# MartijnAB/guacamole

Hardware: AMD Instinct MI355X
Metric: pileup loci/sec at 30x WGS; achieved HBM GB/s vs roofline (higher is better)
Workload: dtype u8; 1 GPU; germline-threshold, synthetic 30x chr20-length shard per GPU (configs[1]); genome_loci=63025519, visited_loci_per_gpu=63025483, reads_per_gpu=12612887, contigs_per_gpu=1, read_len=150, threshold=8, parallelism=loci-sharded x1

## Files before the change

### guacamole_amd/csrc/gq_bamdev.hip

```cpp
#include <hip/hip_runtime.h>
#include <hipcub/hipcub.hpp>

#include <fcntl.h>
#include <sys/mman.h>
#include <sys/stat.h>
#include <unistd.h>

#include <zlib.h>

#include <chrono>
#include <climits>
#include <cstring>
#include <atomic>
#include <map>
#include <memory>
#include <mutex>
#include <string>
#include <thread>
#include <vector>

#include "gq_host.h"

using namespace gq;

// ... 1756 lines not shown
  (void)rehops;
  b->scanned = true;
  *sizes = b->sizes;
  return GQ_OK;
}

gq_status gq_bam_dev_reads(gq_bam_dev *b, const uint8_t *class_sample, int32_t n_samples, const uint32_t *sample_hash,
                           gq_dev_reads **out, float *fill_ms) {
  if (!b || !class_sample || !out) return set_err(GQ_E_ARG, "gq_bam_dev_reads: null argument");
  if (!b->scanned) return set_err(GQ_E_ARG, "gq_bam_dev_reads before gq_bam_dev_scan");
  if (n_samples < 1 || n_samples > 8) return set_err(GQ_E_ARG, "n_samples must be in [1, 8]");
  gq_ctx *c = b->ctx;
  HIP_TRY(hipSetDevice(c->device));
  auto t0 = std::chrono::steady_clock::now();
  const int64_t n = b->n_keep;
  const int32_t n_ref = (int32_t)b->names.size();
  if (n_ref <= 0) return set_err(GQ_E_ARG, "bad read-set sizes");
  std::unique_ptr<gq_dev_reads> dr(new gq_dev_reads());
  gq_dev_reads *d = dr.get();
  d->ctx = c;
  auto alloc = [&](size_t bytes, void **p) -> hipError_t {
    *p = nullptr;
    hipError_t e = hipMalloc(p, std::max(bytes, (size_t)16));
    if (e == hipSuccess) d->owned.push_back(*p);
    return e;
  };
  struct Guard {
    gq_dev_reads *d;
    ~Guard() {
      if (d)
        for (void *p : d->owned) (void)hipFree(p);
    }
  } guard{d};
  FillOut F{};
  void *p;
  DevBuf contig, ekey, cls, tmp, flag;
  const size_t n0 = (size_t)std::max<int64_t>(n, 1);
  HIP_TRY(contig.ensure(sizeof(int32_t) * n0));
  HIP_TRY(ekey.ensure(sizeof(uint64_t) * n0));
  F.contig = (int32_t *)contig.p;
  F.end_key = (uint64_t *)ekey.p;
  HIP_TRY(alloc(sizeof(int32_t) * n0, &p)); F.start = (int32_t *)p;
  HIP_TRY(alloc(sizeof(int32_t) * n0, &p)); F.end = (int32_t *)p;
  HIP_TRY(alloc(n0, &p)); F.mapq = (uint8_t *)p;
  HIP_TRY(alloc(n0, &p)); F.flags = (uint8_t *)p;
  HIP_TRY(alloc(n0, &p)); F.sample = (uint8_t *)p;
  HIP_TRY(alloc(sizeof(int64_t) * n0, &p)); F.seq_off = (int64_t *)p;
  HIP_TRY(alloc(sizeof(int32_t) * n0, &p)); F.seq_len = (int32_t *)p;
  HIP_TRY(alloc(sizeof(int64_t) * n0, &p)); F.cigar_off = (int64_t *)p;
  HIP_TRY(alloc(sizeof(int32_t) * n0, &p)); F.n_cigar = (int32_t *)p;
  HIP_TRY(alloc(sizeof(int64_t) * n0, &p)); F.md_off = (int64_t *)p;
  HIP_TRY(alloc(sizeof(int32_t) * n0, &p)); F.n_md = (int32_t *)p;
  HIP_TRY(alloc(sizeof(uint16_t) * n0, &p)); F.n_mismatch = (uint16_t *)p;
  HIP_TRY(alloc((size_t)b->seq_bytes + kSeqPad, &p)); F.seq = (uint8_t *)p;
  HIP_TRY(hipMemsetAsync(F.seq + b->seq_bytes, 0, kSeqPad, c->stream));
  HIP_TRY(alloc((size_t)b->seq_bytes + kSeqPad, &p)); F.qual = (uint8_t *)p;
  HIP_TRY(hipMemsetAsync(F.qual + b->seq_bytes, 0, kSeqPad, c->stream));
  HIP_TRY(alloc(sizeof(uint32_t) * (size_t)std::max<int64_t>(b->cigar_len, 1), &p)); F.cigar = (uint32_t *)p;
  HIP_TRY(alloc(sizeof(uint32_t) * (size_t)std::max<int64_t>(b->md_events, 1), &p)); F.md_ev = (uint32_t *)p;
  int32_t *pmax;
  HIP_TRY(alloc(sizeof(int32_t) * n0, &p)); pmax = (int32_t *)p;
  int64_t *begin;
  HIP_TRY(alloc(sizeof(int64_t) * (size_t)(n_ref + 1), &p)); begin = (int64_t *)p;
  const int n_cls = 256;
  HIP_TRY(cls.ensure(n_cls));
  HIP_TRY(hipMemsetAsync(cls.p, 0, n_cls, c->stream));
  HIP_TRY(hipMemcpyAsync(cls.p, class_sample, 255, hipMemcpyHostToDevice, c->stream));
  if (b->n_rec) {
    hipLaunchKernelGGL(rec_fill, dim3(grid(b->n_rec * 16, 256)), dim3(256), 0, c->stream, (const uint8_t *)b->out.p,
                       (const int64_t *)b->rec.p, b->n_rec, (const RecInfo *)b->info.p, (const int64_t *)b->kidx.p,
                       (const int64_t *)b->seq_o.p, (const int64_t *)b->cig_o.p, (const int64_t *)b->md_o.p,
                       (const uint8_t *)cls.p, F);
    HIP_TRY(hipGetLastError());
  }
  HIP_TRY(flag.ensure(sizeof(int)));
  HIP_TRY(hipMemsetAsync(flag.p, 0, sizeof(int), c->stream));
  hipLaunchKernelGGL(reads_order, dim3(grid(n + 1, 256)), dim3(256), 0, c->stream, (const int32_t *)F.contig,
                     (const int32_t *)F.start, n, n_ref, begin, (int *)flag.p);
  HIP_TRY(hipGetLastError());
  if (n) {
    size_t tb = 0;
    HIP_TRY(hipcub::DeviceScan::InclusiveScan(nullptr, tb, F.end_key, F.end_key, U64Max(), (int)n, c->stream));
    HIP_TRY(tmp.ensure(tb));
    HIP_TRY(hipcub::DeviceScan::InclusiveScan(tmp.p, tb, F.end_key, F.end_key, U64Max(), (int)n, c->stream));
    hipLaunchKernelGGL(low32, dim3(grid(n, 256)), dim3(256), 0, c->stream, (const uint64_t *)F.end_key, n, pmax);
    HIP_TRY(hipGetLastError());
  }
  int unsorted = 0;
  d->contig_read_begin.assign((size_t)n_ref + 1, 0);
  HIP_TRY(hipMemcpyAsync(&unsorted, flag.p, sizeof(int), hipMemcpyDeviceToHost, c->stream));
  HIP_TRY(hipMemcpyAsync(d->contig_read_begin.data(), begin, sizeof(int64_t) * (size_t)(n_ref + 1),
                         hipMemcpyDeviceToHost, c->stream));
  HIP_TRY(hipStreamSynchronize(c->stream));
  if (unsorted)
    return set_err(GQ_E_UNSORTED, "the BAM's kept reads are not sorted by (contig, start) (the host loader sorts them)");
  DevReads &R = d->d;
  R.n_reads = n;
  R.n_contigs = n_ref;
  R.n_samples = n_samples;
  R.contig_read_begin = begin;
  R.start = F.start;
  R.end = F.end;
  R.pmax_end = pmax;
  R.mapq = F.mapq;
  R.flags = F.flags;
  R.sample = F.sample;
  R.seq_off = F.seq_off;
  R.seq_len = F.seq_len;
  R.cigar_off = F.cigar_off;
  R.n_cigar = F.n_cigar;
  R.md_off = F.md_off;
  R.n_md = F.n_md;
  R.n_mismatch = F.n_mismatch;
  R.seq = F.seq;
  R.qual = F.qual;
  R.cigar = F.cigar;
  R.md_ev = F.md_ev;
  R.seq_bytes = b->seq_bytes;
  R.seq_cap = b->seq_bytes + kSeqPad;
  R.cigar_len = b->cigar_len;
  R.md_len = b->md_events;
  if (sample_hash) {
    HIP_TRY(alloc(sizeof(uint32_t) * (size_t)n_samples, &p));
    HIP_TRY(hipMemcpy(p, sample_hash, sizeof(uint32_t) * (size_t)n_samples, hipMemcpyHostToDevice));
    R.sample_hash = (const uint32_t *)p;
  }
  d->seq_bytes = b->seq_bytes;
  contig.release();
  ekey.release();
  const float fill = ms_since(t0);
  d->h2d_ms = b->sizes.h2d_ms;
  const auto t1 = std::chrono::steady_clock::now();
  gq_status st = derive_shape(c, d, b->md_events);
  d->derive_ms = ms_since(t1);
  if (st) return st;
  if (fill_ms) *fill_ms = fill;
  guard.d = nullptr;
  *out = dr.release();
  return GQ_OK;
}

gq_status gq_reads_positions(const gq_dev_reads *r, int32_t *start, int32_t *end) {
  if (!r || (!start && !end)) return set_err(GQ_E_ARG, "gq_reads_positions: null argument");
  const size_t n = (size_t)r->d.n_reads;
  if (n == 0) return GQ_OK;
  HIP_TRY(hipSetDevice(r->ctx->device));
  if (start) HIP_TRY(hipMemcpyAsync(start, r->d.start, sizeof(int32_t) * n, hipMemcpyDeviceToHost, r->ctx->stream));
  if (end) HIP_TRY(hipMemcpyAsync(end, r->d.end, sizeof(int32_t) * n, hipMemcpyDeviceToHost, r->ctx->stream));
  HIP_TRY(hipStreamSynchronize(r->ctx->stream));
  return GQ_OK;
}

gq_status gq_reads_contig_begin(const gq_dev_reads *r, int64_t *out) {
  if (!r || !out) return set_err(GQ_E_ARG, "gq_reads_contig_begin: null argument");
  std::copy(r->contig_read_begin.begin(), r->contig_read_begin.end(), out);
  return GQ_OK;
}

gq_status gq_reads_download(const gq_dev_reads *r, const gq_reads *dst) {
  if (!r || !dst) return set_err(GQ_E_ARG, "gq_reads_download: null argument");
  HIP_TRY(hipSetDevice(r->ctx->device));
  const DevReads &R = r->d;
  const size_t n = (size_t)R.n_reads;
  hipStream_t st = r->ctx->stream;
  auto cp = [&](const void *h, const void *dv, size_t bytes) -> hipError_t {
    if (!h || !dv || !bytes) return hipSuccess;
    return hipMemcpyAsync(const_cast<void *>(h), dv, bytes, hipMemcpyDeviceToHost, st);
  };
  HIP_TRY(cp(dst->contig_read_begin, R.contig_read_begin, sizeof(int64_t) * (size_t)(R.n_contigs + 1)));
  HIP_TRY(cp(dst->start, R.start, sizeof(int32_t) * n));
  HIP_TRY(cp(dst->end, R.end, sizeof(int32_t) * n));
  HIP_TRY(cp(dst->pmax_end, R.pmax_end, sizeof(int32_t) * n));
// ... 29 lines not shown
```

### guacamole_amd/csrc/gq_germline_direct.h

```cpp
#pragma once

#include "gq_kernels.h"


#ifndef GQ_DIR_WPE
#define GQ_DIR_WPE 4
#endif
#ifndef GQ_DIR_MASKED
#define GQ_DIR_MASKED 0
#endif
#ifndef GQ_DIR_EVPF
#define GQ_DIR_EVPF 0
#endif
#ifndef GQ_DIR_U
#define GQ_DIR_U 4
#endif
struct DirCfg {
  static constexpr int kT = 512;
  static constexpr int kWaves = 4;
  static constexpr int kThreads = 64 * kWaves;
  static constexpr int kU = GQ_DIR_U;
  static constexpr int kRound = 64;
  static constexpr int kSlots = 256;
  static constexpr int64_t kMaxWin = 65535;
// ... 141 lines not shown
      hx[lane] = -1;
      hn[lane] = 0x7FFFFFFF;
      int32_t nslot = 0;
      while (c0 < re) {
        const uint64_t t_rd = (dbg & 16) ? __builtin_readcyclecounter() : 0;
        const int64_t r = c0 + lane;
        const bool valid = r < re;
        const Fields f = nf;
        const int32_t s = f.s, e = f.e, nmd = f.nmd, ld = f.ld;
        const int64_t so = f.so, mo = f.mo;
        const bool nomd = valid && nmd < 0;
        const bool gen = valid && !nomd && ld < 0;
        uint32_t nrun = valid && !nomd && !gen && e > B0 && s < B0 + T ? 1u : 0u;
        const bool evr = valid && !nomd && nmd > 0 && s < B0 + T && !(dbg & 64);
        uint32_t v4[4] = {0u, 0u, 0u, 0u};
        auto load_ev = [&](int32_t k0) {
#pragma unroll
          for (int j = 0; j < 4; ++j) v4[j] = R.md_ev[mo + (k0 + j < nmd ? k0 + j : nmd - 1)];
        };
        auto ev_add = [&](int32_t l, uint8_t base) {
          const int cat = base_cat(base);
          if (cat < 4) {
            const int32_t x = ix(l - B0);
            if (DEEP) atomicAdd(&ev[(cat >> 1) * T + x], 1u << (16 * (cat & 1)));
            else atomicAdd(&ev[x], 1u << (8 * cat));
          }
        };
        if (evr) {
          if (GQ_DIR_EVPF && pv_c0 == c0) {
#pragma unroll
            for (int j = 0; j < 4; ++j) v4[j] = pv4[j];
          } else {
            load_ev(0);
          }
        }
        if (gen && e > B0 && s < B0 + T) nrun = (uint32_t)min(-1 - ld, C::kSlots);
        const uint32_t incl = wave_incl_scan(nrun);
        const int32_t total = (int32_t)__builtin_amdgcn_readlane((int)incl, 63);
        const uint64_t t_f = (dbg & 16) ? __builtin_readcyclecounter() : 0;
        if (nslot > 0 && nslot + total > C::kSlots) break;
        if (total > C::kSlots) {
          bad = true;
          c0 = re;
          break;
        }
        if (c0 + C::kRound < re) nf = load_fields(c0 + C::kRound);
        if (first_round) {
          int64_t so_min = valid ? so : INT64_MAX;
#pragma unroll
          for (int d = 1; d < 64; d <<= 1) {
            const int64_t o = __shfl_xor(so_min, d, 64);
            so_min = o < so_min ? o : so_min;
          }
          defer = !DEEP && so_min < 8;
          tbase = so_min >= 8 ? so_min - 8 : 0;
          tbase = (int64_t)(((uint64_t)(uint32_t)__builtin_amdgcn_readfirstlane((int)(uint32_t)((uint64_t)tbase >> 32)) << 32) |
                            (uint32_t)__builtin_amdgcn_readfirstlane((int)(uint32_t)(uint64_t)tbase));
          const int64_t span = R.seq_cap - tbase;
          srs = __builtin_amdgcn_make_buffer_rsrc((void *)(R.seq + tbase), (short)0,
                                                  (int)(span < 0x7FFFFFFF ? span : 0x7FFFFFFF), 0x00020000);
          first_round = false;
        }
        bad = bad || nomd ||
              (valid && (so < tbase || so + (ld > 0 ? ld : 0) + (e > s ? e - s : 0) + 16384 + 1024 - tbase >= 0x7FFFFFF0ll));
        int32_t slot = nslot + (int32_t)(incl - nrun);
        auto put = [&](int32_t a, int32_t b, int64_t p) {
          const int32_t s16 = min(max(a - B0, -32768), 32767), e16 = min(max(b - B0, -32768), 32767);
          const int32_t K = (int32_t)(p - tbase - (int64_t)(a - B0));
          rc[slot] = make_uint2((uint32_t)(uint16_t)s16 | ((uint32_t)(uint16_t)e16 << 16), (uint32_t)K);
          atomicMax(&hx[min(max(s16, 0), T - 1) >> 3], slot);
          atomicMin(&hn[min(max(e16 - 1, 0), T - 1) >> 3], slot);
          ++slot;
        };
        if (nrun && !gen) put(s, e, so + (ld > 0 ? ld : 0));
        if (gen && e > B0 && s < B0 + T) {
          const int32_t slot_end = slot + (int32_t)nrun;
          const bool ok = general_segments(R, r, [&](uint32_t kind, int32_t ro, int32_t len, int32_t sp, int32_t) {
            const int32_t a = s + ro, b = a + len;
            if (b <= B0 || a >= B0 + T) return;
            if (kind == kSegCount) {
              if (slot < slot_end) put(a, b, so + sp);
              else bad = true;
              if (evr) {
                const int32_t x0 = a > B0 ? a : B0, x1 = b < B0 + T ? b : B0 + T;
#pragma unroll
                for (int j = 0; j < 4; ++j) {
                  const int32_t l = s + (int32_t)(v4[j] >> 8);
                  if (j < nmd && l >= x0 && l < x1) ev_add(l, R.seq[so + sp + (l - a)]);
                }
                for (int32_t k = 4; k < nmd; ++k) {
                  const int32_t l = s + (int32_t)(R.md_ev[mo + k] >> 8);
                  if (l >= x1) break;
                  if (l >= x0) ev_add(l, R.seq[so + sp + (l - a)]);
                }
              }
            } else {
              const bool mid = kind == kSegMidDel;
              uint32_t *dw = mid ? dl : mk;
              const int32_t x0 = a > B0 ? a : B0, x1 = b < B0 + T ? b : B0 + T;
              atomicAdd(&dw[ix(x0 - B0)], mid ? 1u : 1u << 16);
              if (x1 < B0 + T) atomicAdd(&dw[ix(x1 - B0)], mid ? 0xFFFFFFFFu : 0xFFFF0000u);
            }
          });
          bad = bad || !ok;
          for (; slot < slot_end; ++slot) rc[slot] = make_uint2(0u, 0u);
        }
        if (dbg & 16) {
          const uint64_t t_g = __builtin_readcyclecounter();
// ... 287 lines not shown
```

### guacamole_amd/csrc/gq_host.h

```cpp
#pragma once
#include <hip/hip_runtime.h>

#include <algorithm>
#include <cstddef>
#include <cstring>
#include <condition_variable>
#include <mutex>
#include <thread>
#include <cstdarg>
#include <cstdio>
#include <string>
#include <utility>
#include <vector>

#include "../../include/gqpileup.h"
#include "gq_kernels.h"

namespace gq {

gq_status set_err(gq_status s, const char *fmt, ...);

#define HIP_TRY(expr)                                                                         \
  do {                                                                                        \
    hipError_t _e = (expr);                                                                   \
    if (_e != hipSuccess)                                                                     \
      return set_err(GQ_E_HIP, "%s failed: %s (%s:%d)", #expr, hipGetErrorString(_e), __FILE__, __LINE__); \
  } while (0)

constexpr int kBlock = 256;
constexpr int kGermT = 512;
constexpr int kCountT = 512;
constexpr size_t kSeqPad = 2048;

constexpr int kSpread = 64;
constexpr int kPartsCols = 2048;
constexpr int kPartsWalk = 1024;
constexpr int kParts = kPartsCols + kPartsWalk;

struct Counters {
  unsigned long long n_rec;
  unsigned long long n_complex;
  unsigned long long visited;
  unsigned long long ambiguous;
  unsigned long long ties;
  unsigned long long pool_used;
  int err;
  int pad;
  long long err_pos;
  unsigned long long n_slow;
  unsigned long long n_dead;
  unsigned long long part_max[2];
  unsigned long long n_amb;
  unsigned long long n_ord;
  unsigned long long n_deep;
  unsigned long long n_wide;
  unsigned long long n_gdeep[3];
  unsigned long long deep_max;
  unsigned long long deep_nt;
  unsigned long long n_out;
  unsigned long long out_pool;
  unsigned long long spread[4][64];
  unsigned long long prof[8];
  unsigned long long part[2][kParts];
  unsigned long long part_off[2][kParts + 1];
};
constexpr size_t kCountersHead = offsetof(Counters, part);

__device__ __forceinline__ unsigned long long wave_reserve(unsigned long long *ctr, unsigned n) {
  if (__ballot(n != 0) == 0) return 0;
  const int lane = threadIdx.x & 63;
  unsigned x = n;
#pragma unroll
  for (int d = 1; d < 64; d <<= 1) {
    unsigned y = __shfl_up(x, d, 64);
    if (lane >= d) x += y;
  }
  const unsigned total = __shfl(x, 63, 64);
  unsigned long long base = 0;
  if (lane == 63 && total) base = atomicAdd(ctr, (unsigned long long)total);
  base = __shfl(base, 63, 64);
  return base + (x - n);
}

struct OutGeom {
  int ncols;
// ... 973 lines not shown
```

### guacamole_amd/csrc/gq_kernels.h

```cpp
#pragma once
#include <hip/hip_runtime.h>
#include <stdint.h>

#include <type_traits>

namespace gq {

enum : int { OP_M = 0, OP_I = 1, OP_D = 2, OP_N = 3, OP_S = 4, OP_H = 5, OP_P = 6, OP_EQ = 7, OP_X = 8 };

__device__ __forceinline__ bool consumes_ref(int op) {
  return op == OP_M || op == OP_D || op == OP_N || op == OP_EQ || op == OP_X;
}
__device__ __forceinline__ bool consumes_read(int op) {
  return op == OP_M || op == OP_I || op == OP_S || op == OP_EQ || op == OP_X;
}

enum : int { K_SNV = 0, K_INS = 1, K_DEL = 2, K_MID = 3, K_CLIP = 4 };

struct DevReads {
  int64_t n_reads;
  int32_t n_contigs, n_samples;
  const int64_t *contig_read_begin;
  const int32_t *start, *end, *pmax_end;
  const uint8_t *mapq, *flags, *sample;
  const int64_t *seq_off;
  const int32_t *seq_len;
  const int64_t *cigar_off;
  const int32_t *n_cigar;
  const int64_t *md_off;
  const int32_t *n_md;
  const uint16_t *n_mismatch;
  const uint8_t *seq, *qual;
  const uint32_t *cigar, *md_ev;
  int64_t seq_bytes;
  int64_t seq_cap;
  int64_t cigar_len, md_len;
  const int16_t *lead;
  const uint8_t *ev_rb;
  const uint8_t *clean;
  int32_t pool_ordered;
  const struct ColDesc *cdesc;
  const uint32_t *cev;
  const int64_t *caux_off;
  const struct ProjRec *prec;
  const uint8_t *proj;
  const int64_t *qoff;
  const int64_t *srow;
  const uint2 *pev;
  const int64_t *pev_off;
  const uint8_t *pbad;
  const int64_t *sra;
  const int64_t *soff;
  const uint16_t *prow;
  const int64_t *blk_rb, *blk_rs;
  const uint32_t *sample_hash;
};

struct ProjRec {
  int32_t col0, col1;
};
static_assert(sizeof(ProjRec) == 8, "ProjRec layout");
constexpr int32_t kProjNone = (int32_t)0x80000000;
constexpr int kProjRowBytes = 64;
constexpr int kRowPad = 4;
constexpr int32_t kSliceRowsMax = 2048;
constexpr uint32_t kPevComplex = 0x80000000u;
constexpr uint32_t kPevMidDel = 0x40000000u;
constexpr uint32_t kPevLenMask = 0x3FFFFFFFu;
constexpr uint32_t kPevNone = 7u << 4;

struct ColDesc {
  int32_t start, end, pmax_end;
  uint32_t info;
  uint32_t seq_lo;
  uint32_t md_lo;
};
static_assert(sizeof(ColDesc) == 24, "ColDesc layout");
constexpr uint32_t kColEligible = 1u << 16;
constexpr uint32_t kColGeneral = 1u << 17;

struct Tile {
  int64_t ordinal0;
  int64_t rb, re;
  int32_t contig, L0, L1, range;
  int64_t sb0;
  int32_t sbytes;
  int32_t mcnt;
  union {
// ... 358 lines not shown
```

### guacamole_amd/csrc/gq_pileup.hip

```cpp
#include <hip/hip_runtime.h>
#include <hipcub/hipcub.hpp>

#include <algorithm>
#include <chrono>
#include <cstdarg>
#include <cstdlib>
#include <cstdio>
#include <cstring>
#include <string>
#include <thread>
#include <vector>

#include "../../include/gqpileup.h"
#include "gq_host.h"
#include "gq_alleles.h"

using namespace gq;

namespace {
constexpr int kScanT = 256, kScanV = 16, kScanTile = kScanT * kScanV;

__device__ __forceinline__ void scan_load16(const uint32_t *__restrict__ in, int64_t n, int64_t i0, uint32_t (&v)[kScanV]) {
  if (i0 + kScanV <= n) {
    const uint4 *p = reinterpret_cast<const uint4 *>(in + i0);
// ... 57 lines not shown
#pragma unroll
  for (int k = 0; k < kScanV; ++k) x += v[k];
  int64_t run = base[blockIdx.x] + block_excl_i64(x, lds, nullptr);
  int64_t o[kScanV];
#pragma unroll
  for (int k = 0; k < kScanV; ++k) {
    o[k] = run;
    run += v[k];
  }
  if (i0 + kScanV <= n) {
    int4 *q = reinterpret_cast<int4 *>(out + i0);
#pragma unroll
    for (int k = 0; k < kScanV / 2; ++k)
      q[k] = make_int4((int)(uint32_t)o[2 * k], (int)(uint32_t)((uint64_t)o[2 * k] >> 32), (int)(uint32_t)o[2 * k + 1],
                       (int)(uint32_t)((uint64_t)o[2 * k + 1] >> 32));
  } else {
#pragma unroll
    for (int k = 0; k < kScanV; ++k)
      if (i0 + k < n) out[i0 + k] = o[k];
  }
}
}

static hipError_t scan_u32_to_i64(DerivedPool &dp, const uint32_t *in, int64_t *out, int64_t n, hipStream_t st) {
  if (n <= 0) return hipSuccess;
  const int64_t nt = (n + kScanTile - 1) / kScanTile;
  void *sums = nullptr;
  hipError_t e = dp.get(&sums, sizeof(int64_t) * (size_t)nt);
  if (e != hipSuccess) return e;
  hipLaunchKernelGGL(scan_tile_sums, dim3((unsigned)nt), dim3(kScanT), 0, st, in, n, (int64_t *)sums);
  hipLaunchKernelGGL(scan_sums_excl, dim3(1), dim3(kScanT), 0, st, (int64_t *)sums, nt);
  hipLaunchKernelGGL(scan_tiles, dim3((unsigned)nt), dim3(kScanT), 0, st, in, n, (const int64_t *)sums, out);
  e = hipGetLastError();
  dp.put(sums);
  return e;
}

namespace gq {
thread_local std::string g_err;

gq_status set_err(gq_status s, const char *fmt, ...) {
  char buf[1024];
  va_list ap;
  va_start(ap, fmt);
  vsnprintf(buf, sizeof buf, fmt, ap);
  va_end(ap);
  g_err = buf;
  return s;
}

}

namespace {
__global__ void block_index(DevReads R, int64_t n_blocks, int64_t *__restrict__ blk_rb, int64_t *__restrict__ blk_rs) {
  const int64_t g = (int64_t)blockIdx.x * blockDim.x + threadIdx.x;
  if (g >= n_blocks) return;
  int lo = 0, hi = R.n_contigs - 1;
  while (lo < hi) {
    const int m = (lo + hi + 1) >> 1;
    if ((R.qoff[m] >> 2) <= g) lo = m;
    else hi = m - 1;
  }
  const int c = lo;
  const int64_t blk = (g - (R.qoff[c] >> 2)) * 512;
  const int64_t b = R.contig_read_begin[c], e = R.contig_read_begin[c + 1];
  int64_t a0 = b, a1 = e;
  while (a0 < a1) {
    const int64_t m = (a0 + a1) >> 1;
    if ((int64_t)R.pmax_end[m] > blk) a1 = m;
    else a0 = m + 1;
  }
  blk_rb[g] = a0;
  a1 = e;
  while (a0 < a1) {
    const int64_t m = (a0 + a1) >> 1;
    if ((int64_t)R.start[m] >= blk) a1 = m;
    else a0 = m + 1;
  }
  blk_rs[g] = a0;
}

__global__ void plan_tiles(const int32_t *__restrict__ r_contig, const int64_t *__restrict__ r_start,
                           const int64_t *__restrict__ r_end, const int64_t *__restrict__ r_ord,
                           const int64_t *__restrict__ r_tile0, int64_t n_ranges, int64_t n_tiles, int T,
                           DevReads R, Tile *__restrict__ tiles, int stage_cap, int meta_cap, int ev_cap,
                           int aligned, TileX *__restrict__ tilex) {
  const int64_t t = (int64_t)blockIdx.x * blockDim.x + threadIdx.x;
  if (t >= n_tiles) return;
  int64_t lo = 0, hi = n_ranges - 1;
  while (lo < hi) {
    int64_t mid = (lo + hi + 1) >> 1;
    if (r_tile0[mid] <= t) lo = mid;
    else hi = mid - 1;
  }
  const int64_t r = lo;
  const int64_t blk = (r_start[r] / T + (t - r_tile0[r])) * (int64_t)T;
  const int64_t L0 = aligned ? max(r_start[r], blk) : r_start[r] + (t - r_tile0[r]) * (int64_t)T;
  const int64_t L1 = aligned ? min(blk + (int64_t)T, r_end[r]) : min(L0 + (int64_t)T, r_end[r]);
  const int32_t c = r_contig[r];
  int64_t b = R.contig_read_begin[c], e = R.contig_read_begin[c + 1];
  const int64_t W0 = aligned ? blk : L0;
  int64_t a0 = b, a1 = e;
  const int64_t g0 = aligned && T == 512 && R.blk_rb ? (R.qoff[c] >> 2) + blk / 512 : -1, g1 = aligned ? (R.qoff[c + 1] >> 2) : -1;
  if (g0 >= 0) {
    if (g0 >= g1) {
      a0 = a1 = e;
    } else {
      a0 = R.blk_rb[g0];
      a1 = g0 + 1 < g1 ? R.blk_rs[g0 + 1] : e;
      if (L1 < blk + (int64_t)T) {
        int64_t s0 = max(a0, R.blk_rs[g0]);
        while (s0 < a1) {
          int64_t m = (s0 + a1) >> 1;
          if ((int64_t)R.start[m] >= L1) a1 = m;
          else s0 = m + 1;
        }
      }
    }
  } else {
    while (a0 < a1) {
      int64_t m = (a0 + a1) >> 1;
      if ((int64_t)R.pmax_end[m] > W0) a1 = m;
      else a0 = m + 1;
    }
  }
  const int64_t rb = a0;
  if (g0 >= 0) {
    a0 = a1;
  } else {
    a0 = rb;
    a1 = e;
    while (a0 < a1) {
// ... 523 lines not shown
__global__ void ev_bases(DevReads R, uint8_t *__restrict__ ev_rb) {
  const int64_t r = (int64_t)blockIdx.x * blockDim.x + threadIdx.x;
  if (r >= R.n_reads) return;
  const int32_t nmd = R.n_md[r];
  if (nmd <= 0) return;
  const int64_t mdo = R.md_off[r];
  const uint32_t *ev = R.md_ev + mdo;
  uint8_t *rb = ev_rb + mdo;
  const int32_t ld = R.lead[r];
  if (ld >= 0) {
    const int64_t so = R.seq_off[r];
    const int32_t mlen = R.end[r] - R.start[r];
    for (int k0 = 0; k0 < nmd; k0 += 4) {
      uint32_t o4[4];
#pragma unroll
      for (int j = 0; j < 4; ++j) o4[j] = ev[k0 + j < nmd ? k0 + j : nmd - 1] >> 8;
      uint8_t b4[4];
#pragma unroll
      for (int j = 0; j < 4; ++j) {
        const bool in = (int32_t)o4[j] < mlen;
        b4[j] = R.seq[in ? so + ld + (int32_t)o4[j] : so];
        b4[j] = in ? b4[j] : (uint8_t)0;
      }
#pragma unroll
      for (int j = 0; j < 4; ++j)
        if (k0 + j < nmd) rb[k0 + j] = b4[j];
    }
    return;
  }
  const int64_t off = R.cigar_off[r];
  const int32_t n = R.n_cigar[r];
  int32_t ref = 0, rp = 0;
  int k = 0;
  for (int c = 0; c < n && k < nmd; ++c) {
    const uint32_t cc = R.cigar[off + c];
    const int op = (int)(cc & 15u);
    const int32_t len = (int32_t)(cc >> 4);
    if (consumes_ref(op)) {
      while (k < nmd && (int32_t)(ev[k] >> 8) < ref + len) {
        const int32_t o = (int32_t)(ev[k] >> 8);
        uint8_t v = 0;
        if ((op == OP_M || op == OP_EQ || op == OP_X) && o >= ref) {
          const int32_t q = rp + (o - ref);
          if (q < R.seq_len[r]) v = R.seq[R.seq_off[r] + q];
        }
        rb[k++] = v;
      }
      ref += len;
    }
    if (consumes_read(op)) rp += len;
  }
  for (; k < nmd; ++k) rb[k] = 0;
}
__global__ void read_prep(DevReads R, int *__restrict__ bad, int16_t *__restrict__ lead) {
  const int64_t r = (int64_t)blockIdx.x * blockDim.x + threadIdx.x;
  if (r >= R.n_reads) return;
  const int b = validate_one(R, r);
  if (b) atomicOr(bad, b);
  shape_one(R, r, lead, (b & 2) != 0);
}

__device__ __forceinline__ uint64_t pack_inline(uint8_t r0, const uint8_t *alt, int alt_len) {
  uint64_t v = r0;
  for (int i = 0; i < alt_len; ++i) v |= (uint64_t)alt[i] << (8 * (1 + i));
  return v;
}


#include "gq_germline_common.h"
#include "gq_germline_proj.h"
#include "gq_germline_direct.h"
#include "gq_winorder.h"


struct DeepList {
  int64_t *out;
  unsigned long long *n_out;
  const int64_t *sel;
  const unsigned long long *n_sel;
  unsigned long long cap;
};

#ifndef GQ_CPLX_WPE
#define GQ_CPLX_WPE 3
#endif
template <int NS>
__global__ __launch_bounds__(kBlock) __attribute__((amdgpu_waves_per_eu(NS > 2 ? 1 : GQ_CPLX_WPE))) void germline_complex(const Tile *__restrict__ tiles,
                                                           const ComplexItem *__restrict__ items, DevReads R,
                                                           int threshold, int emit_ref, int emit_no_call,
                                                           CallRec *__restrict__ recs, OutGeom og,
                                                           uint8_t *__restrict__ pool, unsigned long long pool_cap,
                                                           Counters *ctr, AmbItem *__restrict__ amb_out,
                                                           unsigned long long amb_cap,
                                                           const AmbItem *__restrict__ amb_in,
                                                           const uint8_t *__restrict__ amb_ref, int64_t n_amb_in,
                                                           int dbg, SomWin sw, DeepList dl) {
  const int lane = threadIdx.x & 63;
  const int64_t gwave = wave_id();
  const int64_t nwaves_total = ((int64_t)gridDim.x * blockDim.x) >> 6;
  const unsigned long long n_list = amb_in ? (unsigned long long)n_amb_in : ctr->part_off[1][kParts];
  const unsigned long long n_items = dl.sel ? min(*dl.n_sel, dl.cap) : n_list;
  const int rpart = kPartsCols + (int)(gwave & (kPartsWalk - 1));
  constexpr int kCover = 256;
  __shared__ int32_t cover_buf[kBlock / 64][kCover];
  int32_t *cover = cover_buf[threadIdx.x >> 6];
  uint64_t clk[6] = {0, 0, 0, 0, 0, 0}, tk = 0;
  auto tick = [&](int k) {
    if (dbg & 32) {
      const uint64_t t = __builtin_readcyclecounter();
      if (k >= 0) clk[k] += t - tk;
      tk = t;
    }
// ... 926 lines not shown
  if (t != 512) return set_err(GQ_E_ARG, "tile must be 512 (the germline column kernel's geometry)");
  c->germ_tile = t;
  return GQ_OK;
}

static gq_status validate_reads(const gq_reads *h) {
  if (!h) return set_err(GQ_E_ARG, "null read set");
  if (h->n_reads < 0 || h->n_contigs <= 0) return set_err(GQ_E_ARG, "bad read-set sizes");
  if (h->n_samples < 1 || h->n_samples > 8) return set_err(GQ_E_ARG, "n_samples must be in [1, 8]");
  return GQ_OK;
}

static gq_status settle_stats(gq_dev_reads *d) {
  if (d->pending & 1) {
    HIP_TRY(hipEventSynchronize(d->tev[1]));
    (void)hipEventElapsedTime(&d->derive_dev_ms, d->tev[0], d->tev[1]);
    const gq_status vs = gq::validation_settled(d);
    if (vs) return vs;
  }
  if (d->pending & 2) {
    HIP_TRY(hipEventSynchronize(d->tev[5]));
    (void)hipEventElapsedTime(&d->fill_ms, d->tev[3], d->tev[4]);
    (void)hipEventElapsedTime(&d->proj_dev_ms, d->tev[2], d->tev[5]);
    std::vector<unsigned long long> hk(kOkSpread);
    HIP_TRY(hipMemcpy(hk.data(), d->nok, sizeof(unsigned long long) * kOkSpread, hipMemcpyDeviceToHost));
    d->proj_reads = 0;
    for (unsigned long long x : hk) d->proj_reads += (int64_t)x;
    d->dp.put(d->nok);
    d->nok = nullptr;
  }
  d->pending = 0;
  return GQ_OK;
}

static gq_status derive_shape_impl(gq_ctx *c, gq_dev_reads *d, int64_t md_len, bool lazy = false) {
  for (hipEvent_t &e : d->tev)
    if (!e) HIP_TRY(hipEventCreate(&e));
  HIP_TRY(hipEventRecord(d->tev[0], c->stream));
  {
    const auto &b = d->contig_read_begin;
    bool ok = !b.empty() && b.front() == 0 && b.back() == d->d.n_reads;
    for (size_t i = 1; i < b.size() && ok; ++i) ok = b[i] >= b[i - 1];
    if (!ok) return set_err(GQ_E_UNSORTED, "contig_read_begin must run from 0 to n_reads, non-decreasing");
  }
  void *p = nullptr;
  HIP_TRY(d->dp.get(&p, sizeof(int16_t) * (size_t)std::max<int64_t>(d->d.n_reads, 1)));
  d->d.lead = (const int16_t *)p;
  d->d.ev_rb = nullptr;
  d->ev_bases = false;
  int unordered = 0;
  const int nc = d->d.n_contigs;
  const bool reuse = lazy && d->shape_kept;
  std::vector<int32_t> last((size_t)nc, 0);
  if (d->d.n_reads > 0) {
    void *flag = nullptr;
    HIP_TRY(d->dp.get(&flag, sizeof(int)));
    HIP_TRY(hipMemsetAsync(flag, 0, sizeof(int), c->stream));
    const unsigned nb = (unsigned)((d->d.n_reads + kBlock - 1) / kBlock);
    hipLaunchKernelGGL(read_prep, dim3(nb), dim3(kBlock), 0, c->stream, d->d, (int *)flag, (int16_t *)p);
    HIP_TRY(hipGetLastError());
    if (reuse) {
      if (!d->vflag) HIP_TRY(hipHostMalloc((void **)&d->vflag, sizeof(int), hipHostMallocDefault));
      *d->vflag = 0;
      HIP_TRY(hipMemcpyAsync(d->vflag, flag, sizeof(int), hipMemcpyDeviceToHost, c->stream));
      d->vflag_pending = true;
      unordered = d->pool_ordered_kept ? 0 : 1;
    } else {
      int bad = 0;
      HIP_TRY(hipMemcpyAsync(&bad, flag, sizeof(int), hipMemcpyDeviceToHost, c->stream));
      const auto &crb = d->contig_read_begin;
      for (int k = 0; k < nc; ++k)
        if (crb[(size_t)k + 1] > crb[(size_t)k])
          HIP_TRY(hipMemcpyAsync(&last[(size_t)k], d->d.pmax_end + (crb[(size_t)k + 1] - 1), sizeof(int32_t),
                                 hipMemcpyDeviceToHost, c->stream));
      HIP_TRY(hipStreamSynchronize(c->stream));
      const gq_status vs = validation_status(bad);
      if (vs) return vs;
      unordered = (bad & 4) ? 1 : 0;
    }
  }
  {
    if (!reuse) {
      std::vector<int64_t> qoff((size_t)nc + 1, 0);
      for (int k = 0; k < nc; ++k) {
        const int64_t col1 = ((int64_t)std::max(last[(size_t)k], 0) + 7) >> 3;
        qoff[(size_t)k + 1] = qoff[(size_t)k] + 4 * ((col1 + 63) >> 6);
      }
      if (!d->qoff_dev) {
        void *qo = nullptr;
        HIP_TRY(hipMalloc(&qo, sizeof(int64_t) * ((size_t)nc + 1)));
        d->owned.push_back(qo);
        d->qoff_dev = (int64_t *)qo;
      }
      HIP_TRY(hipMemcpyAsync(d->qoff_dev, qoff.data(), sizeof(int64_t) * ((size_t)nc + 1), hipMemcpyHostToDevice,
                             c->stream));
      if (lazy) HIP_TRY(hipStreamSynchronize(c->stream));
      d->n_slices_kept = qoff[(size_t)nc];
      d->pool_ordered_kept = unordered ? 0 : 1;
      d->shape_kept = true;
    }
    d->d.qoff = d->qoff_dev;
    d->n_slices = d->n_slices_kept;
    const int64_t n_blk = d->n_slices_kept / 4;
    void *bi = nullptr;
    HIP_TRY(d->dp.get(&bi, sizeof(int64_t) * 2 * (size_t)std::max<int64_t>(n_blk, 1)));
    int64_t *brb = (int64_t *)bi, *brs = brb + std::max<int64_t>(n_blk, 1);
    if (n_blk > 0) {
      hipLaunchKernelGGL(block_index, dim3((unsigned)((n_blk + kBlock - 1) / kBlock)), dim3(kBlock), 0, c->stream, d->d,
                         n_blk, brb, brs);
      HIP_TRY(hipGetLastError());
    }
    d->d.blk_rb = brb;
    d->d.blk_rs = brs;
  }
  HIP_TRY(hipEventRecord(d->tev[1], c->stream));
  d->d.pool_ordered = unordered ? 0 : 1;
  if (lazy) {
    d->pending |= 1;
    return GQ_OK;
  }
  HIP_TRY(hipStreamSynchronize(c->stream));
  (void)hipEventElapsedTime(&d->derive_dev_ms, d->tev[0], d->tev[1]);
  return GQ_OK;
}


gq_status gq_reads_upload(gq_ctx *c, const gq_reads *h, gq_dev_reads **out) {
  if (!c || !out) return set_err(GQ_E_ARG, "gq_reads_upload: null argument");
  gq_status st = validate_reads(h);
  if (st) return st;
  HIP_TRY(hipSetDevice(c->device));
  gq_dev_reads *d = new gq_dev_reads();
  d->ctx = c;
  const int64_t n = h->n_reads;
  const auto t0 = std::chrono::steady_clock::now();
  H2DStager stager(c);
  {
    hipError_t e = stager.init();
    if (e != hipSuccess) {
      delete d;
      return set_err(GQ_E_HIP, "upload: pinned staging: %s", hipGetErrorString(e));
    }
  }
  auto up_from = [&](size_t bytes, void **dst, size_t pad, const auto &src_range) -> hipError_t {
    *dst = nullptr;
    hipError_t e = hipMalloc(dst, std::max(bytes + pad, (size_t)16));
    if (e != hipSuccess) return e;
    d->owned.push_back(*dst);
    if (bytes) e = stager.copy_from(*dst, bytes, src_range);
    if (e == hipSuccess && pad) e = hipMemsetAsync((char *)*dst + bytes, 0, pad, c->stream);
    return e;
  };
  auto up = [&](const void *src, size_t bytes, void **dst, size_t pad) -> hipError_t {
    if (bytes >= (size_t(1) << 20) || (!src && bytes))
      return up_from(bytes, dst, pad, [src](uint8_t *out, size_t o, size_t k) {
        if (src) memcpy(out, (const uint8_t *)src + o, k);
        else memset(out, 0, k);
      });
    *dst = nullptr;
    hipError_t e = hipMalloc(dst, std::max(bytes + pad, (size_t)16));
    if (e != hipSuccess) return e;
    d->owned.push_back(*dst);
    if (bytes) e = hipMemcpyAsync(*dst, src, bytes, hipMemcpyHostToDevice, c->stream);
    if (e == hipSuccess && pad) e = hipMemsetAsync((char *)*dst + bytes, 0, pad, c->stream);
    return e;
  };
  void *p;
#define UP_CHECK(field, T, expr)                                                \
  do {                                                                          \
    hipError_t _e = (expr);                                                     \
    if (_e != hipSuccess) {                                                     \
      gq_reads_free(d);                                                         \
      return set_err(GQ_E_HIP, "upload %s: %s", #field, hipGetErrorString(_e)); \
    }                                                                           \
    d->d.field = (const T *)p;                                                  \
  } while (0)
#define UP(field, count, T) UP_CHECK(field, T, up(h->field, (size_t)(count) * sizeof(T), &p, pad_##field))
  enum : size_t { pad_contig_read_begin = 0, pad_start = 0, pad_end = 0, pad_pmax_end = 0, pad_mapq = 0, pad_flags = 0,
                  pad_sample = 0, pad_seq_off = 0, pad_seq_len = 0, pad_cigar_off = 0, pad_n_cigar = 0, pad_md_off = 0,
                  pad_n_md = 0, pad_n_mismatch = 0, pad_seq = kSeqPad, pad_qual = kSeqPad, pad_cigar = 0,
                  pad_md_ev = 0 };
  const gq_reads *h0 = h;
  gq_reads hh = *h;
  std::vector<int64_t> off2;
  bool ordered = true;
  for (int64_t r = 1; r < n && ordered; ++r) ordered = h->seq_off[r] >= h->seq_off[r - 1] + h->seq_len[r - 1];
  if (!ordered) {
    off2.resize((size_t)n);
    int64_t o = 0;
    for (int64_t r = 0; r < n; ++r) {
      off2[(size_t)r] = o;
      o += h->seq_len[r];
    }
    hh.seq_off = off2.data();
    hh.seq_bytes = o;
  }
  auto gather = [&](const uint8_t *src) {
    return [&, src](uint8_t *out, size_t o, size_t k) {
      if (!src) {
        memset(out, 0, k);
        return;
      }
      int64_t r = (int64_t)(std::upper_bound(off2.begin(), off2.end(), (int64_t)o) - off2.begin()) - 1;
      size_t done = 0;
      while (done < k) {
        const size_t a = o + done - (size_t)off2[(size_t)r];
        const size_t m = std::min((size_t)h0->seq_len[r] - a, k - done);
        memcpy(out + done, src + h0->seq_off[r] + a, m);
        done += m;
        ++r;
      }
    };
  };
  h = &hh;
  UP(contig_read_begin, h->n_contigs + 1, int64_t);
  UP(start, n, int32_t);
  UP(end, n, int32_t);
  UP(pmax_end, n, int32_t);
  UP(mapq, n, uint8_t);
  UP(flags, n, uint8_t);
  UP(sample, n, uint8_t);
  UP(seq_off, n, int64_t);
  UP(seq_len, n, int32_t);
  UP(cigar_off, n, int64_t);
  UP(n_cigar, n, int32_t);
  UP(md_off, n, int64_t);
  UP(n_md, n, int32_t);
  UP(n_mismatch, n, uint16_t);
  if (ordered) {
    UP(seq, h->seq_bytes, uint8_t);
    UP(qual, h->seq_bytes, uint8_t);
  } else {
    UP_CHECK(seq, uint8_t, up_from((size_t)h->seq_bytes, &p, pad_seq, gather(h0->seq)));
    UP_CHECK(qual, uint8_t, up_from((size_t)h->seq_bytes, &p, pad_qual, gather(h0->qual)));
  }
  UP(cigar, h->cigar_len, uint32_t);
  UP(md_ev, h->md_len, uint32_t);
#undef UP
#undef UP_CHECK
  d->d.n_reads = n;
  d->d.seq_bytes = h->seq_bytes;
  d->d.seq_cap = h->seq_bytes + kSeqPad;
  d->d.cigar_len = h->cigar_len;
  d->d.md_len = h->md_len;
  d->d.n_contigs = h->n_contigs;
  d->d.n_samples = h->n_samples;
  if (h->sample_hash && h->n_samples > 0) {
    void *sh = nullptr;
    if (hipMalloc(&sh, sizeof(uint32_t) * (size_t)h->n_samples) != hipSuccess ||
        hipMemcpy(sh, h->sample_hash, sizeof(uint32_t) * (size_t)h->n_samples, hipMemcpyHostToDevice) != hipSuccess) {
      if (sh) (void)hipFree(sh);
      gq_reads_free(d);
      return set_err(GQ_E_HIP, "gq_reads_upload: sample hashes");
    }
    d->owned.push_back(sh);
    d->d.sample_hash = (const uint32_t *)sh;
  }
  d->contig_read_begin.assign(h->contig_read_begin, h->contig_read_begin + h->n_contigs + 1);
  d->seq_bytes = h->seq_bytes;
  if (hipStreamSynchronize(c->stream) != hipSuccess) {
    gq_reads_free(d);
    return set_err(GQ_E_HIP, "gq_reads_upload: copies");
  }
  const auto t1 = std::chrono::steady_clock::now();
  d->h2d_ms = std::chrono::duration<float, std::milli>(t1 - t0).count();
  gq_status st2 = derive_shape_impl(c, d, h->md_len);
  d->derive_ms = std::chrono::duration<float, std::milli>(std::chrono::steady_clock::now() - t1).count();
  if (st2) {
    gq_reads_free(d);
    return st2;
  }
  *out = d;
  return GQ_OK;
}

gq_status gq_reads_wrap_device(gq_ctx *c, const gq_reads *h, gq_dev_reads **out) {
  if (!c || !out) return set_err(GQ_E_ARG, "gq_reads_wrap_device: null argument");
  gq_status st = validate_reads(h);
  if (st) return st;
  gq_dev_reads *d = new gq_dev_reads();
  d->ctx = c;
  d->d.n_reads = h->n_reads;
  d->d.seq_bytes = h->seq_bytes;
  d->d.seq_cap = h->seq_bytes;
  d->d.cigar_len = h->cigar_len;
  d->d.md_len = h->md_len;
  d->d.n_contigs = h->n_contigs;
  d->d.n_samples = h->n_samples;
  d->d.contig_read_begin = h->contig_read_begin;
  d->d.start = h->start;
  d->d.end = h->end;
  d->d.pmax_end = h->pmax_end;
  d->d.mapq = h->mapq;
  d->d.flags = h->flags;
  d->d.sample = h->sample;
  d->d.seq_off = h->seq_off;
  d->d.seq_len = h->seq_len;
  d->d.cigar_off = h->cigar_off;
  d->d.n_cigar = h->n_cigar;
  d->d.md_off = h->md_off;
  d->d.n_md = h->n_md;
  d->d.n_mismatch = h->n_mismatch;
  d->d.seq = h->seq;
  d->d.qual = h->qual;
  d->d.cigar = h->cigar;
  d->d.md_ev = h->md_ev;
  d->d.sample_hash = h->sample_hash;
  d->contig_read_begin.resize((size_t)h->n_contigs + 1);
  hipError_t e = hipMemcpy(d->contig_read_begin.data(), h->contig_read_begin,
                           sizeof(int64_t) * ((size_t)h->n_contigs + 1), hipMemcpyDeviceToHost);
  if (e != hipSuccess) {
    delete d;
    return set_err(GQ_E_HIP, "wrap: contig_read_begin D2H: %s", hipGetErrorString(e));
  }
  d->seq_bytes = h->seq_bytes;
  const auto t1 = std::chrono::steady_clock::now();
  gq_status st2 = derive_shape_impl(c, d, h->md_len);
  d->derive_ms = std::chrono::duration<float, std::milli>(std::chrono::steady_clock::now() - t1).count();
  if (st2) {
    gq_reads_free(d);
    return st2;
  }
  *out = d;
  return GQ_OK;
}

gq_status gq_reads_rederive(gq_ctx *c, gq_dev_reads *d) {
  if (!c || !d) return set_err(GQ_E_ARG, "gq_reads_rederive: null argument");
  if (d->ctx != c) return set_err(GQ_E_ARG, "gq_reads_rederive: the read set belongs to another context");
  HIP_TRY(hipSetDevice(c->device));
  HIP_TRY(hipStreamSynchronize(c->stream));
  HIP_TRY(hipStreamSynchronize(c->side));
  d->nok = nullptr;
  d->pending = 0;
  d->dp.release_all();
  DevReads &R = d->d;
  R.lead = nullptr;
// ... 1005 lines not shown
```

Before: 37.19 billion loci/s.

## Add zeroed seq head padding and fuse block index with read prep

Allocates a small zeroed head region before the device seq buffer so the germline direct kernel can set tbase below offset 8 without falling back to the deferred path. In the reuse path it also fuses block_index and read_prep into one derive_reads launch, saving a kernel launch. The cost is extra allocation and memsets plus a new seq_head field in DevReads, and wrapped device reads keep the old behaviour.

```diff
diff --git a/guacamole_amd/csrc/gq_bamdev.hip b/guacamole_amd/csrc/gq_bamdev.hip
--- a/guacamole_amd/csrc/gq_bamdev.hip
+++ b/guacamole_amd/csrc/gq_bamdev.hip
@@ -1832,7 +1832,8 @@
   HIP_TRY(alloc(sizeof(int64_t) * n0, &p)); F.md_off = (int64_t *)p;
   HIP_TRY(alloc(sizeof(int32_t) * n0, &p)); F.n_md = (int32_t *)p;
   HIP_TRY(alloc(sizeof(uint16_t) * n0, &p)); F.n_mismatch = (uint16_t *)p;
-  HIP_TRY(alloc((size_t)b->seq_bytes + kSeqPad, &p)); F.seq = (uint8_t *)p;
+  HIP_TRY(alloc(kSeqHead + (size_t)b->seq_bytes + kSeqPad, &p)); F.seq = (uint8_t *)p + kSeqHead;
+  HIP_TRY(hipMemsetAsync(p, 0, kSeqHead, c->stream));
   HIP_TRY(hipMemsetAsync(F.seq + b->seq_bytes, 0, kSeqPad, c->stream));
   HIP_TRY(alloc((size_t)b->seq_bytes + kSeqPad, &p)); F.qual = (uint8_t *)p;
   HIP_TRY(hipMemsetAsync(F.qual + b->seq_bytes, 0, kSeqPad, c->stream));
@@ -1898,6 +1899,7 @@
   R.md_ev = F.md_ev;
   R.seq_bytes = b->seq_bytes;
   R.seq_cap = b->seq_bytes + kSeqPad;
+  R.seq_head = (int32_t)kSeqHead;
   R.cigar_len = b->cigar_len;
   R.md_len = b->md_events;
   if (sample_hash) {
diff --git a/guacamole_amd/csrc/gq_germline_direct.h b/guacamole_amd/csrc/gq_germline_direct.h
--- a/guacamole_amd/csrc/gq_germline_direct.h
+++ b/guacamole_amd/csrc/gq_germline_direct.h
@@ -217,8 +217,9 @@
             const int64_t o = __shfl_xor(so_min, d, 64);
             so_min = o < so_min ? o : so_min;
           }
-          defer = !DEEP && so_min < 8;
-          tbase = so_min >= 8 ? so_min - 8 : 0;
+          const bool headed = R.seq_head >= 8 && so_min >= 0;
+          defer = !DEEP && so_min < 8 && !headed;
+          tbase = so_min >= 8 || headed ? so_min - 8 : 0;
           tbase = (int64_t)(((uint64_t)(uint32_t)__builtin_amdgcn_readfirstlane((int)(uint32_t)((uint64_t)tbase >> 32)) << 32) |
                             (uint32_t)__builtin_amdgcn_readfirstlane((int)(uint32_t)(uint64_t)tbase));
           const int64_t span = R.seq_cap - tbase;
diff --git a/guacamole_amd/csrc/gq_host.h b/guacamole_amd/csrc/gq_host.h
--- a/guacamole_amd/csrc/gq_host.h
+++ b/guacamole_amd/csrc/gq_host.h
@@ -31,6 +31,8 @@
 constexpr int kGermT = 512;
 constexpr int kCountT = 512;
 constexpr size_t kSeqPad = 2048;
+
+constexpr size_t kSeqHead = 16;
 
 constexpr int kSpread = 64;
 constexpr int kPartsCols = 2048;
diff --git a/guacamole_amd/csrc/gq_kernels.h b/guacamole_amd/csrc/gq_kernels.h
--- a/guacamole_amd/csrc/gq_kernels.h
+++ b/guacamole_amd/csrc/gq_kernels.h
@@ -34,6 +34,7 @@
   const uint32_t *cigar, *md_ev;
   int64_t seq_bytes;
   int64_t seq_cap;
+  int32_t seq_head;
   int64_t cigar_len, md_len;
   const int16_t *lead;
   const uint8_t *ev_rb;
diff --git a/guacamole_amd/csrc/gq_pileup.hip b/guacamole_amd/csrc/gq_pileup.hip
--- a/guacamole_amd/csrc/gq_pileup.hip
+++ b/guacamole_amd/csrc/gq_pileup.hip
@@ -133,8 +133,9 @@
 }
 
 namespace {
-__global__ void block_index(DevReads R, int64_t n_blocks, int64_t *__restrict__ blk_rb, int64_t *__restrict__ blk_rs) {
-  const int64_t g = (int64_t)blockIdx.x * blockDim.x + threadIdx.x;
+__device__ __forceinline__ void block_index_body(const DevReads &R, int64_t wg, int64_t n_blocks,
+                                                 int64_t *__restrict__ blk_rb, int64_t *__restrict__ blk_rs) {
+  const int64_t g = wg * blockDim.x + threadIdx.x;
   if (g >= n_blocks) return;
   int lo = 0, hi = R.n_contigs - 1;
   while (lo < hi) {
@@ -159,6 +160,9 @@
     else a0 = m + 1;
   }
   blk_rs[g] = a0;
+}
+__global__ void block_index(DevReads R, int64_t n_blocks, int64_t *__restrict__ blk_rb, int64_t *__restrict__ blk_rs) {
+  block_index_body(R, (int64_t)blockIdx.x, n_blocks, blk_rb, blk_rs);
 }
 
 __global__ void plan_tiles(const int32_t *__restrict__ r_contig, const int64_t *__restrict__ r_start,
@@ -788,12 +792,21 @@
   }
   for (; k < nmd; ++k) rb[k] = 0;
 }
-__global__ void read_prep(DevReads R, int *__restrict__ bad, int16_t *__restrict__ lead) {
-  const int64_t r = (int64_t)blockIdx.x * blockDim.x + threadIdx.x;
+__device__ __forceinline__ void read_prep_body(const DevReads &R, int64_t wg, int *__restrict__ bad,
+                                               int16_t *__restrict__ lead) {
+  const int64_t r = wg * blockDim.x + threadIdx.x;
   if (r >= R.n_reads) return;
   const int b = validate_one(R, r);
   if (b) atomicOr(bad, b);
   shape_one(R, r, lead, (b & 2) != 0);
+}
+__global__ void read_prep(DevReads R, int *__restrict__ bad, int16_t *__restrict__ lead) {
+  read_prep_body(R, (int64_t)blockIdx.x, bad, lead);
+}
+__global__ void derive_reads(DevReads R, unsigned n_blk_wg, int64_t n_blocks, int64_t *__restrict__ blk_rb,
+                             int64_t *__restrict__ blk_rs, int *__restrict__ bad, int16_t *__restrict__ lead) {
+  if (blockIdx.x < n_blk_wg) block_index_body(R, (int64_t)blockIdx.x, n_blocks, blk_rb, blk_rs);
+  else read_prep_body(R, (int64_t)(blockIdx.x - n_blk_wg), bad, lead);
 }
 
 __device__ __forceinline__ uint64_t pack_inline(uint8_t r0, const uint8_t *alt, int alt_len) {
@@ -1826,32 +1839,51 @@
   const int nc = d->d.n_contigs;
   const bool reuse = lazy && d->shape_kept;
   std::vector<int32_t> last((size_t)nc, 0);
-  if (d->d.n_reads > 0) {
-    void *flag = nullptr;
+  int64_t n_blk = 0, *brb = nullptr, *brs = nullptr;
+  auto index_buffers = [&]() -> hipError_t {
+    n_blk = d->n_slices_kept / 4;
+    void *bi = nullptr;
+    const hipError_t e = d->dp.get(&bi, sizeof(int64_t) * 2 * (size_t)std::max<int64_t>(n_blk, 1));
+    brb = (int64_t *)bi;
+    brs = brb + std::max<int64_t>(n_blk, 1);
+    return e;
+  };
+  void *flag = nullptr;
+  const unsigned nb = (unsigned)((d->d.n_reads + kBlock - 1) / kBlock);
+  if (nb) {
     HIP_TRY(d->dp.get(&flag, sizeof(int)));
     HIP_TRY(hipMemsetAsync(flag, 0, sizeof(int), c->stream));
-    const unsigned nb = (unsigned)((d->d.n_reads + kBlock - 1) / kBlock);
-    hipLaunchKernelGGL(read_prep, dim3(nb), dim3(kBlock), 0, c->stream, d->d, (int *)flag, (int16_t *)p);
-    HIP_TRY(hipGetLastError());
-    if (reuse) {
+  }
+  if (reuse) {
+    d->d.qoff = d->qoff_dev;
+    HIP_TRY(index_buffers());
+    const unsigned n_blk_wg = (unsigned)((n_blk + kBlock - 1) / kBlock);
+    if (n_blk_wg + nb) {
+      hipLaunchKernelGGL(derive_reads, dim3(n_blk_wg + nb), dim3(kBlock), 0, c->stream, d->d, n_blk_wg, n_blk, brb, brs,
+                         (int *)flag, (int16_t *)p);
+      HIP_TRY(hipGetLastError());
+    }
+    if (nb) {
       if (!d->vflag) HIP_TRY(hipHostMalloc((void **)&d->vflag, sizeof(int), hipHostMallocDefault));
       *d->vflag = 0;
       HIP_TRY(hipMemcpyAsync(d->vflag, flag, sizeof(int), hipMemcpyDeviceToHost, c->stream));
       d->vflag_pending = true;
       unordered = d->pool_ordered_kept ? 0 : 1;
-    } else {
-      int bad = 0;
-      HIP_TRY(hipMemcpyAsync(&bad, flag, sizeof(int), hipMemcpyDeviceToHost, c->stream));
-      const auto &crb = d->contig_read_begin;
-      for (int k = 0; k < nc; ++k)
-        if (crb[(size_t)k + 1] > crb[(size_t)k])
-          HIP_TRY(hipMemcpyAsync(&last[(size_t)k], d->d.pmax_end + (crb[(size_t)k + 1] - 1), sizeof(int32_t),
-                                 hipMemcpyDeviceToHost, c->stream));
-      HIP_TRY(hipStreamSynchronize(c->stream));
-      const gq_status vs = validation_status(bad);
-      if (vs) return vs;
-      unordered = (bad & 4) ? 1 : 0;
-    }
+    }
+  } else if (nb) {
+    hipLaunchKernelGGL(read_prep, dim3(nb), dim3(kBlock), 0, c->stream, d->d, (int *)flag, (int16_t *)p);
+    HIP_TRY(hipGetLastError());
+    int bad = 0;
+    HIP_TRY(hipMemcpyAsync(&bad, flag, sizeof(int), hipMemcpyDeviceToHost, c->stream));
+    const auto &crb = d->contig_read_begin;
+    for (int k = 0; k < nc; ++k)
+      if (crb[(size_t)k + 1] > crb[(size_t)k])
+        HIP_TRY(hipMemcpyAsync(&last[(size_t)k], d->d.pmax_end + (crb[(size_t)k + 1] - 1), sizeof(int32_t),
+                               hipMemcpyDeviceToHost, c->stream));
+    HIP_TRY(hipStreamSynchronize(c->stream));
+    const gq_status vs = validation_status(bad);
+    if (vs) return vs;
+    unordered = (bad & 4) ? 1 : 0;
   }
   {
     if (!reuse) {
@@ -1875,14 +1907,13 @@
     }
     d->d.qoff = d->qoff_dev;
     d->n_slices = d->n_slices_kept;
-    const int64_t n_blk = d->n_slices_kept / 4;
-    void *bi = nullptr;
-    HIP_TRY(d->dp.get(&bi, sizeof(int64_t) * 2 * (size_t)std::max<int64_t>(n_blk, 1)));
-    int64_t *brb = (int64_t *)bi, *brs = brb + std::max<int64_t>(n_blk, 1);
-    if (n_blk > 0) {
-      hipLaunchKernelGGL(block_index, dim3((unsigned)((n_blk + kBlock - 1) / kBlock)), dim3(kBlock), 0, c->stream, d->d,
-                         n_blk, brb, brs);
-      HIP_TRY(hipGetLastError());
+    if (!reuse) {
+      HIP_TRY(index_buffers());
+      if (n_blk > 0) {
+        hipLaunchKernelGGL(block_index, dim3((unsigned)((n_blk + kBlock - 1) / kBlock)), dim3(kBlock), 0, c->stream, d->d,
+                           n_blk, brb, brs);
+        HIP_TRY(hipGetLastError());
+      }
     }
     d->d.blk_rb = brb;
     d->d.blk_rs = brs;
@@ -1916,25 +1947,32 @@
       return set_err(GQ_E_HIP, "upload: pinned staging: %s", hipGetErrorString(e));
     }
   }
-  auto up_from = [&](size_t bytes, void **dst, size_t pad, const auto &src_range) -> hipError_t {
+  auto alloc_head = [&](size_t bytes, void **dst, size_t head) -> hipError_t {
     *dst = nullptr;
-    hipError_t e = hipMalloc(dst, std::max(bytes + pad, (size_t)16));
+    hipError_t e = hipMalloc(dst, std::max(head + bytes, (size_t)16));
     if (e != hipSuccess) return e;
     d->owned.push_back(*dst);
+    if (head) {
+      e = hipMemsetAsync(*dst, 0, head, c->stream);
+      *dst = (char *)*dst + head;
+    }
+    return e;
+  };
+  auto up_from = [&](size_t bytes, void **dst, size_t pad, size_t head, const auto &src_range) -> hipError_t {
+    hipError_t e = alloc_head(bytes + pad, dst, head);
+    if (e != hipSuccess) return e;
     if (bytes) e = stager.copy_from(*dst, bytes, src_range);
     if (e == hipSuccess && pad) e = hipMemsetAsync((char *)*dst + bytes, 0, pad, c->stream);
     return e;
   };
-  auto up = [&](const void *src, size_t bytes, void **dst, size_t pad) -> hipError_t {
+  auto up = [&](const void *src, size_t bytes, void **dst, size_t pad, size_t head) -> hipError_t {
     if (bytes >= (size_t(1) << 20) || (!src && bytes))
-      return up_from(bytes, dst, pad, [src](uint8_t *out, size_t o, size_t k) {
+      return up_from(bytes, dst, pad, head, [src](uint8_t *out, size_t o, size_t k) {
         if (src) memcpy(out, (const uint8_t *)src + o, k);
         else memset(out, 0, k);
       });
-    *dst = nullptr;
-    hipError_t e = hipMalloc(dst, std::max(bytes + pad, (size_t)16));
+    hipError_t e = alloc_head(bytes + pad, dst, head);
     if (e != hipSuccess) return e;
-    d->owned.push_back(*dst);
     if (bytes) e = hipMemcpyAsync(*dst, src, bytes, hipMemcpyHostToDevice, c->stream);
     if (e == hipSuccess && pad) e = hipMemsetAsync((char *)*dst + bytes, 0, pad, c->stream);
     return e;
@@ -1949,7 +1987,9 @@
     }                                                                           \
     d->d.field = (const T *)p;                                                  \
   } while (0)
-#define UP(field, count, T) UP_CHECK(field, T, up(h->field, (size_t)(count) * sizeof(T), &p, pad_##field))
+#define UP_HEAD(field, count, T, head) \
+  UP_CHECK(field, T, up(h->field, (size_t)(count) * sizeof(T), &p, pad_##field, head))
+#define UP(field, count, T) UP_HEAD(field, count, T, 0)
   enum : size_t { pad_contig_read_begin = 0, pad_start = 0, pad_end = 0, pad_pmax_end = 0, pad_mapq = 0, pad_flags = 0,
                   pad_sample = 0, pad_seq_off = 0, pad_seq_len = 0, pad_cigar_off = 0, pad_n_cigar = 0, pad_md_off = 0,
                   pad_n_md = 0, pad_n_mismatch = 0, pad_seq = kSeqPad, pad_qual = kSeqPad, pad_cigar = 0,
@@ -2002,19 +2042,21 @@
   UP(n_md, n, int32_t);
   UP(n_mismatch, n, uint16_t);
   if (ordered) {
-    UP(seq, h->seq_bytes, uint8_t);
+    UP_HEAD(seq, h->seq_bytes, uint8_t, kSeqHead);
     UP(qual, h->seq_bytes, uint8_t);
   } else {
-    UP_CHECK(seq, uint8_t, up_from((size_t)h->seq_bytes, &p, pad_seq, gather(h0->seq)));
-    UP_CHECK(qual, uint8_t, up_from((size_t)h->seq_bytes, &p, pad_qual, gather(h0->qual)));
+    UP_CHECK(seq, uint8_t, up_from((size_t)h->seq_bytes, &p, pad_seq, kSeqHead, gather(h0->seq)));
+    UP_CHECK(qual, uint8_t, up_from((size_t)h->seq_bytes, &p, pad_qual, 0, gather(h0->qual)));
   }
   UP(cigar, h->cigar_len, uint32_t);
   UP(md_ev, h->md_len, uint32_t);
 #undef UP
+#undef UP_HEAD
 #undef UP_CHECK
   d->d.n_reads = n;
   d->d.seq_bytes = h->seq_bytes;
   d->d.seq_cap = h->seq_bytes + kSeqPad;
+  d->d.seq_head = (int32_t)kSeqHead;
   d->d.cigar_len = h->cigar_len;
   d->d.md_len = h->md_len;
   d->d.n_contigs = h->n_contigs;
@@ -2057,6 +2099,7 @@
   d->d.n_reads = h->n_reads;
   d->d.seq_bytes = h->seq_bytes;
   d->d.seq_cap = h->seq_bytes;
+  d->d.seq_head = 0;
   d->d.cigar_len = h->cigar_len;
   d->d.md_len = h->md_len;
   d->d.n_contigs = h->n_contigs;
```

Result: faster. 38.46 billion loci/s, median of 6 (+3.4%).
